# tho-kn/EgoTAP

Measured on AMD Instinct MI355X. Metric: stereo frames/sec (2D->3D lift, B=256, 256x256), higher is better.
Workload: dtype f32; 1 GPU; UnrealEgo 16-joint lifting head (heatmaps [B,90,64,64] -> joints [B,16,3]), forward only, fp32, batch 256 per GPU, inputs resident in HBM; batch_per_gpu=256, global_batch=256, heatmap=64, parallelism=dp1 (batch shards, no collective)

## Files before the change

egotap_amd/csrc/egotap_abi.hip:

```cpp
#include <stdarg.h>
#include <stdio.h>
#include <string.h>

#include <string>
#include <unordered_map>
#include <vector>

#include "attention_f32.h"
#include "common.h"
#include "conv_f32.h"
#include "conv_bf16.h"
#include "gemm_f32.h"
#include "gemm_bf16.h"
#include "gemm_bf16_dma.h"
#include "gemm_f32_dma.h"
#include "attention_bf16.h"
#include "layernorm.h"
#include "metrics.h"
#include "heatmap_synth.h"
#include "pu_chain.h"
#include "gemm_tn_bf16.h"
#include "train_ops.h"
#include "gemm_bf16s.h"
#include "gemm_bf16s64.h"
// ... 773 lines not shown
static hipError_t launch_ln(const float* x, float* y, const float* g, const float* b, int rows, float eps, hipStream_t s) {
    if (rows <= 0) return hipSuccess;
    const int blocks = min((rows + 3) / 4, 256 * 8);
    hipLaunchKernelGGL(layernorm_f32_kernel<1024>, dim3(blocks), dim3(256), 0, s, x, y, g, b, rows, eps);
    return hipGetLastError();
}

#if EGOTAP_IN(0)
static hipError_t gemm_res_ln(Handle* h, const char* role, const float* A, long lda, const float* Wp, const float* bias, float* X, int M, int D, int K,
                              const float* ln_g, const float* ln_b, float* Y, float* P, hipStream_t s) {
    if (D == 1024) {
        const SmallRoute r = gemm_small_route(h, true, M, D, K, D, device_cu_count());
        if ((r.kind == GS_SPLIT_S || r.kind == GS_SPLIT_A) && r.splits > 1) {
            static const std::string kname = "gemm_f32_splitk_kernel<ALoadPlain>+splitk_reduce_res_ln_kernel";
            GemmTimer t(h, s, role, kname.c_str(), 2.0 * M * D * K);
            hipError_t e = r.kind == GS_SPLIT_S ? gemm_f32_splitk_partials<TileS>(ALoadPlain{A, lda}, segmat1(Wp, D, K), P, SPLITK_FLOATS, M, D, K, s, r.splits)
                                                : gemm_f32_splitk_partials<TileA>(ALoadPlain{A, lda}, segmat1(Wp, D, K), P, SPLITK_FLOATS, M, D, K, s, r.splits);
            if (e != hipSuccess) return e;
            hipLaunchKernelGGL(splitk_reduce_res_ln_kernel<1024>, dim3(min((M + 3) / 4, 256 * 8)), dim3(256), 0, s, (const float*)P, bias, (const float*)X, X, ln_g,
                               ln_b, Y, M, r.splits, 1e-12f);
            return hipGetLastError();
        }
    }
    hipError_t e = gemm_small(h, role, ALoadPlain{A, lda}, segmat1(Wp, D, K), EpiBiasRes{segvec1(bias, D), X, D}, X, D, M, D, K, P, s);
    if (e != hipSuccess) return e;
    return launch_ln(X, Y, ln_g, ln_b, M, 1e-12f, s);
}

static ALoadPlain rebase(const ALoadPlain& a, int m0) { return ALoadPlain{a.A + (long)m0 * a.lda, a.lda}; }
static ALoadLive rebase(ALoadLive a, int m0) { a.lr.m0 += m0; return a; }
static EpiBias rebase(const EpiBias& e, int) { return e; }
static EpiBiasGelu rebase(const EpiBiasGelu& e, int) { return e; }
static EpiBiasRes rebase(EpiBiasRes e, int m0) { e.R += (long)m0 * e.ldr; return e; }
static EpiBiasResLive rebase(EpiBiasResLive e, int m0) { e.lr.m0 += m0; return e; }
template <class AL, class Epi>
static hipError_t gemm_rounds(Handle* h, const char* role, const AL& al, const SegMat& W, const Epi& epi, float* C, long ldc, int M, int N, int K,
                              hipStream_t s) {
    const int cus = device_cu_count(), tn = N / 256;
    const long tiles = (long)((M + 255) / 256) * tn;
    const int mh = (int)((tiles / cus) * cus / tn) * 256;
    if (N % 256 == 0 && K % 32 == 0 && mh > 0 && mh < M) {
        const double t_round = K * 0.2319 + 5.0;
        const double t_big = (double)((tiles + cus - 1) / cus) * t_round;
        const double t_split = (double)(((long)(mh / 256) * tn + cus - 1) / cus) * t_round + 4.0 + gemm_f32_direct_estimate_us<TileA>(M - mh, N, K, cus);
        if (t_split < t_big) {
            hipError_t e = gemm_big(h, role, al, W, epi, C, ldc, mh, N, K, s);
            if (e != hipSuccess) return e;
            return gemm<TileA>(h, role, rebase(al, mh), W, rebase(epi, mh), C + (long)mh * ldc, ldc, M - mh, N, K, s);
        }
    }
    return gemm_big(h, role, al, W, epi, C, ldc, M, N, K, s);
}

static bool lift_prune_last(Handle* h, int B) {
#ifdef EGOTAP_ATTN_F32_LIVE
    const int D = h->D, M = B * h->seq, Nq = h->T * h->ppd * h->ppd;
    if (h->precision != EGOTAP_PREC_F32 || h->debug_stop != 0 || h->cfg.vit_layers < 1 || Nq < 32 || Nq >= h->seq || D % 256 != 0) return false;
    const int cus = device_cu_count();
    if (gemm_small_route(h, true, M, 3 * D, D, D, cus, true).kind != GS_BIG || gemm_small_route(h, true, M, D, D, D, cus).kind != GS_BIG ||
        gemm_small_route(h, true, M, 4 * D, D, 4 * D, cus, true).kind != GS_BIG || gemm_small_route(h, true, M, D, 4 * D, D, cus).kind != GS_BIG)
        return false;
    return attention_f32_ksplit(B, h->seq, h->cfg.vit_heads, SPLITK_FLOATS, cus) == 1;
#else
    (void)h; (void)B;
    return false;
#endif
}

static int lift_forward_impl(Handle* h, const float* hm, int B, float* pose, void* ws, size_t ws_bytes, void* stream, bool pose_only,
                             const char* who) {
    EGO_CHECK(h, "null handle");
    if (B == 0) return EGOTAP_OK;
    EGO_CHECK(B > 0 && hm && pose && ws, "%s: null argument or negative batch", who);
    EGO_CHECK(((uintptr_t)hm & 15) == 0 && ((uintptr_t)ws & 255) == 0, "hm must be 16-byte and ws 256-byte aligned");
    int rc = lift_resolve(h);
    if (rc != EGOTAP_OK) return rc;
    const LiftWs w = lift_ws(h, B);
    if (ws_bytes < w.total) {
        egotap_set_error("workspace too small: %zu bytes given, %zu needed for B=%d", ws_bytes, w.total, B);
        return EGOTAP_ERR_WORKSPACE;
    }
    hipStream_t s = (hipStream_t)stream;
    const LiftParams& p = h->lp;
    char* base = (char*)ws;
    auto F = [&](size_t off) { return (float*)(base + off); };
    float *X = F(w.X), *Y = F(w.Y), *QKV = F(w.QKV), *CTX = F(w.CTX), *HID = F(w.HID);
    float* SPK = F(w.SPLITK);
    float *Z1 = F(w.Z1), *Z2 = F(w.Z2), *POSZ = F(w.POSZ), *ROTZ = F(w.ROTZ);
    float *F0 = F(w.F0), *G0 = F(w.G0), *HS0 = F(w.HS0), *F1 = F(w.F1), *G1 = F(w.G1), *HS1 = F(w.HS1);
    float *C0 = F(w.C0), *C1 = F(w.C1), *ZERO = F(w.ZERO), *HPA = F(w.HPA), *HPB = F(w.HPB);
    const int D = h->D, M = B * h->seq, BT = B * h->T, J = h->J, H = h->H, hid = h->hid, JB = J * B;
    const int S = h->cfg.hm_size, HW = S * S;
    using Tile = TileA;

#ifndef EGOTAP_BF16S_MIN_ROWS
#define EGOTAP_BF16S_MIN_ROWS 512
#endif
    constexpr int g_bf16s_min_rows = EGOTAP_BF16S_MIN_ROWS;
    const bool bf16s = h->precision == EGOTAP_PREC_BF16 && D == 1024 && M >= g_bf16s_min_rows && h->wscratch != nullptr && h->seq % 32 == 0 &&
                       h->wscratch_bytes >= (size_t)2 * 2048 * (size_t)(h->ppd * h->ppd * D);
    if (bf16s) {
        __bf16* hmb0 = (__bf16*)HID;
        const long n8 = (long)B * h->C * HW / 8;
        hipLaunchKernelGGL(f32_to_bf16_kernel, dim3((unsigned)((n8 + 255) / 256)), dim3(256), 0, s, hm, hmb0, n8);
        hipLaunchKernelGGL(prep_weight_kernel, dim3((256 + 63) / 64, (D + 63) / 64), dim3(256), 0, s, p.patch_w, h->wscratch, (__bf16*)nullptr, D, 256, (long)D);
        EGO_HIP(zero_fill(SPK, 256, s));
        const XPatch xl{hmb0, (const __bf16*)SPK, h->C, S, h->seq, h->side, h->ppd, h->grid, h->T};
        const SEpiPatchF32 ep{p.patch_b, p.mask_tok, p.pos_emb, X, D, h->seq, h->side, h->ppd, h->grid, h->T};
        EGO_HIP(gemm_bf16s_launch(xl, h->wscratch, 256L, ep, M, D, 256, device_cu_count(), s));
    } else {
        ALoadPatch al{hm, h->C, S, h->seq, h->side, h->ppd, h->grid, h->T};
        if (h->precision == EGOTAP_PREC_F32 && (long)((M + 255) / 256) * (D / 256) >= 160 && (size_t)B * H * 4 >= 1024) {
            EGO_HIP(zero_fill(ZERO, 1024, s));
            al.zeros = ZERO;
        }
        EpiPatch ep{p.patch_b, p.mask_tok, p.pos_emb, D, h->seq, h->side, h->ppd, h->grid, h->T};
        EGO_HIP((gemm_small(h, "patch_embed", al, segmat1(p.patch_w, D, 256), ep, X, D, M, D, 256, SPK, s)));
    }
    if (h->debug_stop == 1) return EGOTAP_OK;
    if (bf16s) {
        __bf16 *Yb = (__bf16*)Y, *QKVb = (__bf16*)QKV, *CTXb = (__bf16*)CTX, *HIDb = (__bf16*)HID, *Wb = h->wscratch;
        float* bias3 = SPK;
        const int cu = device_cu_count();
        auto prep = [&](const float* wsrc, __bf16* dst, int n, int k) {
            hipLaunchKernelGGL(prep_weight_kernel, dim3((k + 63) / 64, (n + 63) / 64), dim3(256), 0, s, wsrc, dst, (__bf16*)nullptr, n, k, (long)n);
        };
        auto ln = [&](const float* gg, const float* bb) {
            hipLaunchKernelGGL(ln_fwd_bf16_kernel<1024>, dim3((M + 3) / 4), dim3(256), 0, s, (const float*)X, Yb, gg, bb, (float*)nullptr, (float*)nullptr, M, 1e-12f);
        };
        for (int i = 0; i < h->cfg.vit_layers; ++i) {
            const auto& L = p.layer[i];
            ln(L.ln1_g, L.ln1_b);
            prep(L.q_w, Wb, D, D); prep(L.k_w, Wb + (size_t)D * D, D, D); prep(L.v_w, Wb + (size_t)2 * D * D, D, D);
            hipLaunchKernelGGL(concat3_kernel, dim3((D + 255) / 256), dim3(256), 0, s, L.q_b, L.k_b, L.v_b, bias3, D);
            EGO_HIP(hipGetLastError());
            EGO_HIP(gemm_bf16s_plain_launch(XPlain{Yb, (long)D}, Wb, (long)D, SEpiBf16{bias3, QKVb, 3L * D}, M, 3 * D, D, cu, s));
            EGO_HIP(attention_bf16s_fwd_launch(QKVb, CTXb, nullptr, B, h->seq, h->cfg.vit_heads, s));
            prep(L.o_w, Wb, D, D);
            EGO_HIP(gemm_bf16s_plain_launch(XPlain{CTXb, (long)D}, Wb, (long)D, SEpiResF32{L.o_b, X, X, (long)D}, M, D, D, cu, s));
            ln(L.ln2_g, L.ln2_b);
            prep(L.up_w, Wb, 4 * D, D);
            EGO_HIP(gemm_bf16s_plain_launch(XPlain{Yb, (long)D}, Wb, (long)D, SEpiGelu{L.up_b, HIDb, 4L * D}, M, 4 * D, D, cu, s));
            prep(L.dn_w, Wb, D, 4 * D);
            EGO_HIP(gemm_bf16s_plain_launch(XPlain{HIDb, 4L * D}, Wb, 4L * D, SEpiResF32{L.dn_b, X, X, (long)D}, M, D, 4 * D, cu, s));
            if (h->debug_stop == 2 + i) return EGOTAP_OK;
        }
        ln(p.lnf_g, p.lnf_b);
        auto bnf = [](const LiftParams::Fc& f, float* out) { return SEpiBnLreluF32{f.b, f.g, f.beta, f.mean, f.var, 1e-5f, 0.2f, out, 2048L}; };
        auto bn = [](const LiftParams::Fc& f) { return EpiBnLrelu{f.b, f.g, f.beta, f.mean, f.var, 1e-5f, 0.2f}; };
        {
            const int K1 = h->ppd * h->ppd * D;
            prep(p.pos_fc[0].w, Wb, 2048, K1);
            const XTokens xt{Yb, h->T, D, h->seq, h->side, h->ppd, h->grid};
            const int sp = gemm_bf16s_ksplit(BT, 2048, K1, cu, SPLITK_FLOATS);
            if (sp > 1) EGO_HIP(gemm_bf16s_splitk_launch(xt, Wb, (long)K1, bnf(p.pos_fc[0], Z1), SPK, sp, BT, 2048, K1, cu, s));
            else EGO_HIP(fc1_nt(h, 0, Yb, Wb, (long)K1, bnf(p.pos_fc[0], Z1), BT, cu, s));
            EGO_HIP((fc_gemm(h, "pos_fc2", ALoadPlain{Z1, 2048}, segmat1(p.pos_fc[1].w, 512, 2048), bn(p.pos_fc[1]), Z2, 512, BT, 512, 2048, SPK, s)));
            EGO_HIP((fc_gemm(h, "pos_fc3", ALoadPlain{Z2, 512}, segmat1(p.pos_fc[2].w, hid, 512), bn(p.pos_fc[2]), POSZ, hid, BT, hid, 512, SPK, s)));
        }
        {
            __bf16* hmb = HIDb;
            const long n8 = (long)B * h->C * HW / 8;
            hipLaunchKernelGGL(f32_to_bf16_kernel, dim3((unsigned)((n8 + 255) / 256)), dim3(256), 0, s, hm, hmb, n8);
            prep(p.rot_fc[0].w, Wb, 2048, 2 * HW);
            EGO_HIP(hipGetLastError());
            const XRot xr{hmb, h->C, J, HW};
            const int sp = gemm_bf16s_ksplit(BT, 2048, 2 * HW, cu, SPLITK_FLOATS);
            if (sp > 1) EGO_HIP(gemm_bf16s_splitk_launch(xr, Wb, 2L * HW, bnf(p.rot_fc[0], Z1), SPK, sp, BT, 2048, 2 * HW, cu, s));
            else EGO_HIP(fc1_nt(h, 1, hmb, Wb, 2L * HW, bnf(p.rot_fc[0], Z1), BT, cu, s));
            EGO_HIP((fc_gemm(h, "rot_fc2", ALoadPlain{Z1, 2048}, segmat1(p.rot_fc[1].w, 512, 2048), bn(p.rot_fc[1]), Z2, 512, BT, 512, 2048, SPK, s)));
            EGO_HIP((fc_gemm(h, "rot_fc3", ALoadPlain{Z2, 512}, segmat1(p.rot_fc[2].w, hid, 512), bn(p.rot_fc[2]), ROTZ, hid, BT, hid, 512, SPK, s)));
        }
    } else {
    const int NL = h->cfg.vit_layers;
    const bool prune = pose_only && lift_prune_last(h, B);
    EGO_HIP(launch_ln(X, Y, NL > 0 ? p.layer[0].ln1_g : p.lnf_g, NL > 0 ? p.layer[0].ln1_b : p.lnf_b, M, 1e-12f, s));
    for (int i = 0; i < NL; ++i) {
        const auto& L = p.layer[i];
#ifdef EGOTAP_ATTN_F32_LIVE
        if (prune && i + 1 == NL) {
            const LiveRows lr{h->seq, h->side, h->ppd, h->grid, h->T};
            const int Nq = h->T * h->ppd * h->ppd, Mc = B * Nq;
            float* Xc = QKV;
            SegMat Wkv; Wkv.p[0] = L.k_w; Wkv.p[1] = L.v_w; Wkv.p[2] = L.v_w; Wkv.seg = D; Wkv.ld = D;
            SegVec bkv; bkv.p[0] = L.k_b; bkv.p[1] = L.v_b; bkv.p[2] = L.v_b; bkv.seg = D;
            EGO_HIP((gemm_big(h, "kv", ALoadPlain{Y, D}, Wkv, EpiBias{bkv}, QKV + D, 3L * D, M, 2 * D, D, s)));
            EGO_HIP((gemm_rounds(h, "q_live", ALoadLive{Y, D, lr}, segmat1(L.q_w, D, D), EpiBias{segvec1(L.q_b, D)}, QKV, 3L * D, Mc, D, D, s)));
            EGO_HIP(attention_f32_live_launch(QKV, 3L * D, Nq, QKV, CTX, B, h->seq, h->cfg.vit_heads, s));
            EGO_HIP((gemm_rounds(h, "attn_out_live", ALoadPlain{CTX, D}, segmat1(L.o_w, D, D), EpiBiasResLive{segvec1(L.o_b, D), X, D, lr}, Xc, D, Mc, D, D, s)));
            EGO_HIP(launch_ln(Xc, Y, L.ln2_g, L.ln2_b, Mc, 1e-12f, s));
            EGO_HIP((gemm_rounds(h, "mlp_up_live", ALoadPlain{Y, D}, segmat1(L.up_w, 4 * D, D), EpiBiasGelu{segvec1(L.up_b, 4 * D)}, HID, 4L * D, Mc, 4 * D, D, s)));
            EGO_HIP((gemm_rounds(h, "mlp_down_live", ALoadPlain{HID, 4L * D}, segmat1(L.dn_w, D, 4 * D), EpiBiasRes{segvec1(L.dn_b, D), Xc, D}, Xc, D, Mc, D, 4 * D, s)));
            EGO_HIP(launch_ln(Xc, Y, p.lnf_g, p.lnf_b, Mc, 1e-12f, s));
            break;
        }
#endif
        {
            SegMat Wqkv; Wqkv.p[0] = L.q_w; Wqkv.p[1] = L.k_w; Wqkv.p[2] = L.v_w; Wqkv.seg = D; Wqkv.ld = D;
            SegVec bqkv; bqkv.p[0] = L.q_b; bqkv.p[1] = L.k_b; bqkv.p[2] = L.v_b; bqkv.seg = D;
            EGO_HIP((gemm_small(h, "qkv", ALoadPlain{Y, D}, Wqkv, EpiBias{bqkv}, QKV, 3L * D, M, 3 * D, D, SPK, s)));
        }
        if (h->precision == EGOTAP_PREC_BF16X3 && h->seq % 32 == 0) EGO_HIP(attention_bf16_launch<3>(QKV, CTX, B, h->seq, h->cfg.vit_heads, s));
        else if (h->precision == EGOTAP_PREC_BF16 && h->seq % 32 == 0) EGO_HIP(attention_bf16_launch<1>(QKV, CTX, B, h->seq, h->cfg.vit_heads, s));
        else EGO_HIP(attention_f32_launch(QKV, CTX, B, h->seq, h->cfg.vit_heads, s, nullptr, SPK, SPLITK_FLOATS, device_cu_count()));
        EGO_HIP(gemm_res_ln(h, "attn_out", CTX, D, L.o_w, L.o_b, X, M, D, D, L.ln2_g, L.ln2_b, Y, SPK, s));
        EGO_HIP((gemm_small(h, "mlp_up", ALoadPlain{Y, D}, segmat1(L.up_w, 4 * D, D), EpiBiasGelu{segvec1(L.up_b, 4 * D)}, HID, 4L * D, M, 4 * D, D, SPK, s)));
        const bool last = i + 1 == NL;
        EGO_HIP(gemm_res_ln(h, "mlp_down", HID, 4L * D, L.dn_w, L.dn_b, X, M, D, 4 * D, last ? p.lnf_g : p.layer[i + 1].ln1_g, last ? p.lnf_b : p.layer[i + 1].ln1_b, Y,
                            SPK, s));
        if (h->debug_stop == 2 + i) return EGOTAP_OK;
    }
    auto bn = [](const LiftParams::Fc& f) { return EpiBnLrelu{f.b, f.g, f.beta, f.mean, f.var, 1e-5f, 0.2f}; };
    const bool skinny_fc1 = BT < SKINNY_ROWS || (h->precision == EGOTAP_PREC_F32 && (long)((BT + 255) / 256) * (2048 / 256) < 100);
    {
        const int K1 = h->ppd * h->ppd * D;
        auto fc1 = [&](const auto& al) -> hipError_t {
            if (skinny_fc1 && BT <= 64)
                return gemm_f32_splitk_launch<TileS>(al, segmat1(p.pos_fc[0].w, 2048, K1), bn(p.pos_fc[0]), Z1, 2048, SPK, SPLITK_FLOATS, BT, 2048, K1, s, device_cu_count());
            if (skinny_fc1)
                return gemm_f32_splitk_launch<TileA>(al, segmat1(p.pos_fc[0].w, 2048, K1), bn(p.pos_fc[0]), Z1, 2048, SPK, SPLITK_FLOATS, BT, 2048, K1, s);
            return gemm_big(h, "pos_fc1", al, segmat1(p.pos_fc[0].w, 2048, K1), bn(p.pos_fc[0]), Z1, 2048, BT, 2048, K1, s);
        };
        if (prune) EGO_HIP(fc1(ALoadPlain{Y, (long)K1}));
        else EGO_HIP(fc1(ALoadTokens{Y, h->T, D, h->seq, h->side, h->ppd, h->grid}));
        EGO_HIP((fc_gemm(h, "pos_fc2", ALoadPlain{Z1, 2048}, segmat1(p.pos_fc[1].w, 512, 2048), bn(p.pos_fc[1]), Z2, 512, BT, 512, 2048, SPK, s)));
        EGO_HIP((fc_gemm(h, "pos_fc3", ALoadPlain{Z2, 512}, segmat1(p.pos_fc[2].w, hid, 512), bn(p.pos_fc[2]), POSZ, hid, BT, hid, 512, SPK, s)));
    }
    {
        ALoadRot al{hm, h->C, J, HW};
        if (skinny_fc1 && BT <= 64)
            EGO_HIP((gemm_f32_splitk_launch<TileS>(al, segmat1(p.rot_fc[0].w, 2048, 2L * HW), bn(p.rot_fc[0]), Z1, 2048, SPK, SPLITK_FLOATS, BT, 2048, 2 * HW, s, device_cu_count())));
        else if (skinny_fc1)
            EGO_HIP((gemm_f32_splitk_launch<TileA>(al, segmat1(p.rot_fc[0].w, 2048, 2L * HW), bn(p.rot_fc[0]), Z1, 2048, SPK, SPLITK_FLOATS, BT, 2048, 2 * HW, s)));
        else
            EGO_HIP((gemm_big(h, "rot_fc1", al, segmat1(p.rot_fc[0].w, 2048, 2L * HW), bn(p.rot_fc[0]), Z1, 2048, BT, 2048, 2 * HW, s)));
        EGO_HIP((fc_gemm(h, "rot_fc2", ALoadPlain{Z1, 2048}, segmat1(p.rot_fc[1].w, 512, 2048), bn(p.rot_fc[1]), Z2, 512, BT, 512, 2048, SPK, s)));
        EGO_HIP((fc_gemm(h, "rot_fc3", ALoadPlain{Z2, 512}, segmat1(p.rot_fc[2].w, hid, 512), bn(p.rot_fc[2]), ROTZ, hid, BT, hid, 512, SPK, s)));
    }
    }
    const int x = 2 * hid, NF0 = H + x;
    ALoadStereo xs{POSZ, B, J, hid};
    EGO_HIP((fc_gemm(h, "pu0_x2f", xs, segmat1(p.x2f0_w, NF0, x), EpiBias{segvec1(p.x2f0_b, NF0)}, F0, NF0, JB, NF0, x, SPK, s)));
    EGO_HIP((fc_gemm(h, "pu0_x2h", xs, segmat1(p.x2h0_w, 4 * H, x), EpiBias{segvec1(p.x2h0_b, 4 * H)}, G0, 4L * H, JB, 4 * H, x, SPK, s)));
    {
        ALoadStereoGated bs{ALoadStereo{ROTZ, B, J, hid}, F0, NF0, H};
        EGO_HIP((fc_gemm(h, "pu0_b2h", bs, segmat1(p.b2h0_w, 4 * H, x), EpiBiasRes{segvec1(p.b2h0_b, 4 * H), G0, 4L * H}, G0, 4L * H, JB, 4 * H, x, SPK, s)));
    }
    EGO_HIP(zero_fill(C0, (size_t)(w.ZERO - w.C0) + al256((size_t)B * H * 4), s));
    pu_chain_probe(h);
    unsigned* FAULT = (unsigned*)(base + w.FAULT);
    const PuChain ch0{F0, (long)B * NF0, NF0, G0, (long)B * 4 * H, nullptr, p.h2h0_w, p.h2h0_b, nullptr, 0, HS0, (long)B * H, HPA, (long)B * H, B, H, J,
                      FAULT, h->pu_fault_dev};
    if (!pu_chain_launch(s, h->pu_resident[0], h->pu_resident[1], ch0, B, h->pu_debug_drop))
// ... 2467 lines not shown
```

egotap_amd/csrc/gemm_f32.h:

```cpp
#pragma once
#include "common.h"
#include <type_traits>

struct ALoadPlain {
    const float* A;
    long lda;
    struct Row { const float* p; };
    __device__ __forceinline__ Row row(int m) const { return Row{A + (long)m * lda}; }
    __device__ __forceinline__ f32x4 load(const Row& r, int k) const { return *(const f32x4*)(r.p + k); }
    static constexpr bool HAS_PTR = true;
    __device__ __forceinline__ const float* ptr(const Row& r, int k) const { return r.p + k; }
    __host__ bool dma_ok() const { return lda % 4 == 0 && lda < (1L << 21) && ((uintptr_t)A & 15) == 0; }
};

struct ALoadPatch {
    const float* hm;
    int C, S, seq, side, ppd, grid, T;
    const float* zeros = nullptr;
    struct Row { const float* p; };
    static constexpr bool HAS_PTR = true;
    __device__ __forceinline__ const float* ptr(const Row& r, int k) const { return r.p ? r.p + (k >> 4) * S + (k & 15) : zeros + k; }
    __host__ bool dma_ok() const { return zeros != nullptr && S % 4 == 0 && ((uintptr_t)hm & 15) == 0 && ((uintptr_t)zeros & 15) == 0; }
    __device__ __forceinline__ Row row(int m) const {
        const int b = m / seq, tok = m - b * seq;
// ... 3 lines not shown
        return Row{hm + ((long)(b * C + cell) * S + (pr % ppd) * 16) * S + (pc % ppd) * 16};
    }
    __device__ __forceinline__ f32x4 load(const Row& r, int k) const {
        if (r.p == nullptr) return f32x4{0.f, 0.f, 0.f, 0.f};
        return *(const f32x4*)(r.p + (k >> 4) * S + (k & 15));
    }
};

struct ALoadTokens {
    const float* Y;
    int T, D, seq, side, ppd, grid;
    struct Row { const float* p; };
    __device__ __forceinline__ Row row(int m) const {
        const int b = m / T, i = m - b * T;
        return Row{Y + ((long)b * seq + (long)(ppd * (i / grid)) * side + ppd * (i % grid)) * D};
    }
    __device__ __forceinline__ f32x4 load(const Row& r, int k) const {
        const int s = k / D, c = k - s * D;
        const int prl = s / ppd, pcl = s - prl * ppd;
        return *(const f32x4*)(r.p + (long)(prl * side + pcl) * D + c);
    }
    static constexpr bool HAS_PTR = true;
    __device__ __forceinline__ const float* ptr(const Row& r, int k) const {
        const int s = k / D, c = k - s * D;
        const int prl = s / ppd, pcl = s - prl * ppd;
        return r.p + (long)(prl * side + pcl) * D + c;
    }
    __host__ bool dma_ok() const { return D % 4 == 0 && ((uintptr_t)Y & 15) == 0; }
};

struct LiveRows {
    int seq, side, ppd, grid, T;
    int m0 = 0;
    __host__ __device__ __forceinline__ long phys(int m) const {
        m += m0;
        const int pp = ppd * ppd, L = T * pp;
        const int b = m / L, r = m - b * L, i = r / pp, s = r - i * pp;
        const int pr = (i / grid) * ppd + s / ppd, pc = (i % grid) * ppd + s % ppd;
        return (long)b * seq + pr * side + pc;
    }
};
struct ALoadLive {
    const float* A;
    long lda;
    LiveRows lr;
    struct Row { const float* p; };
    __device__ __forceinline__ Row row(int m) const { return Row{A + lr.phys(m) * lda}; }
    __device__ __forceinline__ f32x4 load(const Row& r, int k) const { return *(const f32x4*)(r.p + k); }
    static constexpr bool HAS_PTR = true;
    __device__ __forceinline__ const float* ptr(const Row& r, int k) const { return r.p + k; }
    __host__ bool dma_ok() const { return lda % 4 == 0 && lda < (1L << 21) && ((uintptr_t)A & 15) == 0; }
};

struct ALoadRot {
    const float* hm;
    int C, J, HW;
    struct Row { const float* p; };
    __device__ __forceinline__ Row row(int m) const {
        const int T = 2 * J;
        const int b = m / T, t = m - b * T;
        const int eye = t / J, j = t - eye * J;
        return Row{hm + (long)(b * C + 2 * J + eye * 2 * J + j) * HW};
    }
    __device__ __forceinline__ f32x4 load(const Row& r, int k) const {
        const int cs = k / HW;
        return *(const f32x4*)(r.p + (long)cs * J * HW + (k - cs * HW));
    }
    static constexpr bool HAS_PTR = true;
    __device__ __forceinline__ const float* ptr(const Row& r, int k) const {
        const int cs = k / HW;
        return r.p + (long)cs * J * HW + (k - cs * HW);
    }
    __host__ bool dma_ok() const { return HW % 4 == 0 && ((uintptr_t)hm & 15) == 0; }
};

struct ALoadStereo {
    static constexpr bool HAS_PTR = false;
    const float* Z;
    int B, J, hid;
    struct Row { const float* p; };
    __device__ __forceinline__ Row row(int m) const {
        const int t = m / B, b = m - t * B;
        return Row{Z + ((long)b * 2 * J + t) * hid};
    }
    __device__ __forceinline__ f32x4 load(const Row& r, int k) const {
        const int eye = k / hid;
        return *(const f32x4*)(r.p + (long)eye * J * hid + (k - eye * hid));
    }
};

struct ALoadStereoGated {
    static constexpr bool HAS_PTR = false;
    ALoadStereo z;
    const float* F;
    int ldf, fcol0;
    struct Row { ALoadStereo::Row r; const float* f; };
    __device__ __forceinline__ Row row(int m) const { return Row{z.row(m), F + (long)m * ldf + fcol0}; }
    __device__ __forceinline__ f32x4 load(const Row& r, int k) const {
        f32x4 v = z.load(r.r, k);
        const f32x4 g = *(const f32x4*)(r.f + k);
#pragma unroll
        for (int i = 0; i < 4; ++i) v[i] *= 1.0f / (1.0f + expf(-g[i]));
        return v;
    }
};

// ... 55 lines not shown
        f32x4 o;
#pragma unroll
        for (int i = 0; i < 4; ++i) {
            const float x = acc[i] + c.b[i];
            o[i] = gelu_erf(x);
        }
        return o;
    }
};
struct EpiBnLrelu {
    const float *bias, *gamma, *beta, *mean, *var;
    float eps, slope;
    struct Col { float b, mu, sc, sh; };
    __device__ __forceinline__ Col col(int n) const {
        return Col{bias[n], mean[n], gamma[n] / sqrtf(var[n] + eps), beta[n]};
    }
    __device__ __forceinline__ float apply(float acc, const Col& c, int m, int n) const {
        const float y = (acc + c.b - c.mu) * c.sc + c.sh;
        return y > 0.f ? y : slope * y;
    }
    struct Col4 { Col c[4]; };
    __device__ __forceinline__ Col4 col4(int n0) const { return Col4{{col(n0), col(n0 + 1), col(n0 + 2), col(n0 + 3)}}; }
    static constexpr bool HAS_RES = false;
    __device__ __forceinline__ f32x4 res4(int m, int n0) const { return f32x4{0.f, 0.f, 0.f, 0.f}; }
    __device__ __forceinline__ f32x4 apply4(f32x4 acc, const Col4& c, f32x4 res, int m, int n0) const {
        f32x4 o;
#pragma unroll
        for (int i = 0; i < 4; ++i) o[i] = apply(acc[i], c.c[i], m, n0 + i);
        return o;
    }
};
struct EpiPatch {
    const float *bias, *mask_tok, *pos;
    int D, seq, side, ppd, grid, T;
    struct Col { float b, mt; };
    __device__ __forceinline__ Col col(int n) const { return Col{bias[n], mask_tok[n]}; }
    __device__ __forceinline__ float apply(float acc, const Col& c, int m, int n) const {
        const int tok = m % seq;
        const int pr = tok / side, pc = tok - pr * side;
        const bool dummy = (pr / ppd) * grid + pc / ppd >= T;
        return (dummy ? c.mt : acc + c.b) + pos[(long)tok * D + n];
    }
    struct Col4 { f32x4 b, mt; };
    __device__ __forceinline__ Col4 col4(int n0) const { return Col4{*(const f32x4*)(bias + n0), *(const f32x4*)(mask_tok + n0)}; }
    static constexpr bool HAS_RES = true;
    __device__ __forceinline__ f32x4 res4(int m, int n0) const { return *(const f32x4*)(pos + (long)(m % seq) * D + n0); }
    __device__ __forceinline__ f32x4 apply4(f32x4 acc, const Col4& c, f32x4 res, int m, int n0) const {
        const int tok = m % seq;
        const int pr = tok / side, pc = tok - pr * side;
        const bool dummy = (pr / ppd) * grid + pc / ppd >= T;
        return (dummy ? c.mt : acc + c.b) + res;
    }
};

struct EpiNone {
    struct Col {};
    __device__ __forceinline__ Col col(int n) const { return Col{}; }
    __device__ __forceinline__ float apply(float acc, const Col& c, int m, int n) const { return acc; }
    struct Col4 {};
    __device__ __forceinline__ Col4 col4(int n0) const { return Col4{}; }
    static constexpr bool HAS_RES = false;
    __device__ __forceinline__ f32x4 res4(int m, int n0) const { return f32x4{0.f, 0.f, 0.f, 0.f}; }
    __device__ __forceinline__ f32x4 apply4(f32x4 acc, const Col4& c, f32x4 res, int m, int n0) const { return acc; }
};
struct EpiAccum {
    const float* R;
    long ldr;
    struct Col {};
    __device__ __forceinline__ Col col(int n) const { return Col{}; }
    __device__ __forceinline__ float apply(float acc, const Col& c, int m, int n) const { return acc + R[(long)m * ldr + n]; }
    struct Col4 {};
    __device__ __forceinline__ Col4 col4(int n0) const { return Col4{}; }
    static constexpr bool HAS_RES = true;
    __device__ __forceinline__ f32x4 res4(int m, int n0) const { return *(const f32x4*)(R + (long)m * ldr + n0); }
    __device__ __forceinline__ f32x4 apply4(f32x4 acc, const Col4& c, f32x4 res, int m, int n0) const { return acc + res; }
};
struct EpiBiasGeluSave {
    SegVec bias;
    float* Z;
    long ldz;
    struct Col { float b; };
    __device__ __forceinline__ Col col(int n) const { return Col{bias.at(n)}; }
    __device__ __forceinline__ float apply(float acc, const Col& c, int m, int n) const {
        const float x = acc + c.b;
        Z[(long)m * ldz + n] = x;
        return gelu_erf(x);
    }
    struct Col4 { f32x4 b; };
    __device__ __forceinline__ Col4 col4(int n0) const { return Col4{bias.at4(n0)}; }
    static constexpr bool HAS_RES = false;
    __device__ __forceinline__ f32x4 res4(int m, int n0) const { return f32x4{0.f, 0.f, 0.f, 0.f}; }
    __device__ __forceinline__ f32x4 apply4(f32x4 acc, const Col4& c, f32x4 res, int m, int n0) const {
        const f32x4 x = acc + c.b;
        *(f32x4*)(Z + (long)m * ldz + n0) = x;
        f32x4 o;
#pragma unroll
        for (int i = 0; i < 4; ++i) o[i] = gelu_erf(x[i]);
        return o;
    }
};
struct EpiGeluGrad {
    const float* Z;
    long ldz;
    __device__ __forceinline__ static float dgelu(float z) {
        return dgelu_erf(z);
    }
// ... 664 lines not shown
```

egotap_amd/csrc/gemm_f32_dma.h:

```cpp
#pragma once
#include <type_traits>
#include "gemm_f32.h"
#include "lds_dma.h"

struct DmaF32Cfg {
    static constexpr int BM = 256, BN = 256, BK = 16, WM = 4, WN = 2, THREADS = 512, NS = 4, TM = 2, TN = 4;
    static constexpr int ROWB = 64;
    static constexpr int STAGE = (BM + BN) * ROWB;
    static constexpr int ELD = 36, EPATCH = 16 * ELD * 4;
    static constexpr int LDS_BYTES = NS * STAGE + (THREADS / 64) * EPATCH;
    static_assert(LDS_BYTES <= 160 * 1024, "LDS budget");
};

template <class ALoad, class Epi>
__global__ __launch_bounds__(DmaF32Cfg::THREADS, 2) void gemm_f32_dma_kernel(ALoad al, SegMat W, Epi epi, float* C,
                                                                          long ldc, int M, int N, int K, int tiles_m, int tiles_n) {
    using Cfg = DmaF32Cfg;
    constexpr int BM = Cfg::BM, BN = Cfg::BN, BK = Cfg::BK, NS = Cfg::NS, TM = Cfg::TM, TN = Cfg::TN, ROWB = Cfg::ROWB, ELD = Cfg::ELD;
    extern __shared__ __attribute__((aligned(16))) char smem_dmaf[];
    const int tid = threadIdx.x, lane = tid & 63, wid = tid >> 6;
    const int wm = wid / Cfg::WN, wn = wid % Cfg::WN;
    const int l31 = lane & 31, lh = lane >> 5;
    float* Es = (float*)(smem_dmaf + NS * Cfg::STAGE + wid * Cfg::EPATCH);

    const int ntiles = tiles_m * tiles_n, nb = gridDim.x, x8 = blockIdx.x & 7, jb = blockIdx.x >> 3;
    const int nbx = (nb >> 3) + (x8 < (nb & 7) ? 1 : 0);
    const int q8 = ntiles >> 3, r8 = ntiles & 7;
    const int lo_t = x8 < r8 ? x8 * (q8 + 1) : r8 * (q8 + 1) + (x8 - r8) * q8;
    const int cnt = q8 + (x8 < r8 ? 1 : 0);
    const int my_n = cnt > jb ? (cnt - jb + nbx - 1) / nbx : 0;
    const int KT = K / BK;
    const int total = my_n * KT;
    if (total == 0) return;
    auto tile_of = [&](int i, int& tm, int& tn) __attribute__((always_inline)) {
        const int lin = lo_t + jb + i * nbx;
        const int per_group = 8 * tiles_n;
        const int g = lin / per_group, first = g * 8;
        const int gsz = min(tiles_m - first, 8);
        const int in = lin - g * per_group;
        tm = first + in % gsz;
        tn = in / gsz;
    };

    const int drow = lane >> 2, dchunk = (lane & 3) ^ (lane >> 4);
    typename ALoad::Row ra0, ra1;
    const float *pb0, *pb1;
#ifdef EGOTAP_F32_DMA_FLAT
    constexpr bool SBA = false, SBW = false;
#else
    constexpr bool SBA = std::is_same<ALoad, ALoadPlain>::value, SBW = true;
#endif
    unsigned long long abase = 0, wbase = 0;
    unsigned ao0 = 0, ao1 = 0;
    auto uniform64 = [](const void* p) __attribute__((always_inline)) { return lds_dma_base(p); };
    const unsigned wo0 = (unsigned)(((long)(wid * 16 + drow) * W.ld + dchunk * 4) * 4), wo1 = (unsigned)(((long)((wid + 8) * 16 + drow) * W.ld + dchunk * 4) * 4);
    int l_tile = 0, l_kt = 0;
    auto set_rows = [&](int i) __attribute__((always_inline)) {
        int tm, tn;
        tile_of(i, tm, tn);
        if constexpr (SBA) {
            abase = uniform64(al.A + (long)tm * BM * al.lda);
            const long ld = al.lda * 4;
            ao0 = (unsigned)((long)(min(tm * BM + wid * 16 + drow, M - 1) - tm * BM) * ld + dchunk * 16);
            ao1 = (unsigned)((long)(min(tm * BM + (wid + 8) * 16 + drow, M - 1) - tm * BM) * ld + dchunk * 16);
        } else {
        ra0 = al.row(min(tm * BM + wid * 16 + drow, M - 1));
        ra1 = al.row(min(tm * BM + (wid + 8) * 16 + drow, M - 1));
        }
        const int n0 = tn * BN, sidx = n0 / W.seg;
        const float* wp = (sidx == 0 ? W.p[0] : (sidx == 1 ? W.p[1] : W.p[2])) + (long)(n0 - sidx * W.seg) * W.ld;
        if constexpr (SBW) wbase = uniform64(wp);
        else {
        pb0 = wp + (long)(wid * 16 + drow) * W.ld + dchunk * 4;
        pb1 = wp + (long)((wid + 8) * 16 + drow) * W.ld + dchunk * 4;
        }
    };
    set_rows(0);
    const unsigned lds0 = (unsigned)(size_t)(__attribute__((address_space(3))) char*)smem_dmaf;
    auto dma1 = [&](const float* g, unsigned lds_addr) __attribute__((always_inline)) {
        asm volatile("s_mov_b32 m0, %1\n\ts_nop 0\n\tglobal_load_lds_dwordx4 %0, off" ::"v"(g), "s"(__builtin_amdgcn_readfirstlane(lds_addr)) : "memory");
    };
    auto dma1s = [&](unsigned voff, unsigned long long sbase, unsigned lds_addr) __attribute__((always_inline)) {
        asm volatile("s_mov_b32 m0, %2\n\ts_nop 0\n\tglobal_load_lds_dwordx4 %0, %1" ::"v"(voff), "s"(sbase), "s"(__builtin_amdgcn_readfirstlane(lds_addr)) : "memory");
    };
    auto dma_part = [&](int st, int part) __attribute__((always_inline)) {
        const unsigned sa = lds0 + st * Cfg::STAGE + wid * 1024;
        const int k0 = l_kt * BK;
        if (part == 0) { if constexpr (SBA) dma1s(ao0, abase + (unsigned long long)k0 * 4, sa); else dma1(al.ptr(ra0, k0 + dchunk * 4), sa); }
        else if (part == 1) { if constexpr (SBA) dma1s(ao1, abase + (unsigned long long)k0 * 4, sa + 8 * 1024); else dma1(al.ptr(ra1, k0 + dchunk * 4), sa + 8 * 1024); }
        else if (part == 2) { if constexpr (SBW) dma1s(wo0, wbase + (unsigned long long)k0 * 4, sa + BM * ROWB); else dma1(pb0 + k0, sa + BM * ROWB); }
        else { if constexpr (SBW) dma1s(wo1, wbase + (unsigned long long)k0 * 4, sa + BM * ROWB + 8 * 1024); else dma1(pb1 + k0, sa + BM * ROWB + 8 * 1024); }
    };
    auto dma_advance = [&]() __attribute__((always_inline)) {
        if (l_tile < my_n && ++l_kt == KT) {
            l_kt = 0;
            if (++l_tile < my_n) set_rows(l_tile);
            else l_kt = KT - 1;
        }
    };
    auto dma = [&](int st) __attribute__((always_inline)) {
        dma_part(st, 0); dma_part(st, 1); dma_part(st, 2); dma_part(st, 3);
        dma_advance();
    };

    f32x16 acc[TM][TN];
#pragma unroll
    for (int i = 0; i < TM; ++i)
#pragma unroll
        for (int j = 0; j < TN; ++j)
#pragma unroll
            for (int r = 0; r < 16; ++r) acc[i][j][r] = 0.f;
    const int sw = (l31 >> 2) & 3;
    const int f0 = l31 * ROWB + ((lh ^ sw) << 4), f1 = l31 * ROWB + (((2 + lh) ^ sw) << 4);
    const int a_base = (wm * (TM * 32)) * ROWB, b_base = (BM + wn * (TN * 32)) * ROWB;

    int c_tile = 0, c_kt = 0;
    auto epilogue = [&](auto full_tag) __attribute__((always_inline)) {
        constexpr bool FULL = decltype(full_tag)::value;
        int tm, tn;
        tile_of(c_tile, tm, tn);
        const int er = lane >> 3, ec = (lane & 7) * 4;
        const int nb0 = tn * BN + wn * (TN * 32) + ec, mb0 = tm * BM + wm * (TM * 32) + er;
        f32x4 rs[2] = {{0.f, 0.f, 0.f, 0.f}, {0.f, 0.f, 0.f, 0.f}}, rn[2] = {{0.f, 0.f, 0.f, 0.f}, {0.f, 0.f, 0.f, 0.f}};
        if (Epi::HAS_RES) {
#pragma unroll
            for (int s2 = 0; s2 < 2; ++s2) rs[s2] = epi.res4(min(mb0 + s2 * 8, M - 1), nb0);
        }
        typename Epi::Col4 cc = epi.col4(nb0), cn = cc;
#pragma unroll
        for (int q = 0; q < TN * TM * 2; ++q) {
            const int j = q / (TM * 2), i = (q / 2) % TM, hf = q & 1;
            const int n0 = nb0 + j * 32, mb = mb0 + i * 32;
            if (q + 1 < TN * TM * 2 && (q + 1) / (TM * 2) != j) cn = epi.col4(nb0 + ((q + 1) / (TM * 2)) * 32);
            if (Epi::HAS_RES && q + 1 < TN * TM * 2) {
                const int jn = (q + 1) / (TM * 2), in = ((q + 1) / 2) % TM, hn = (q + 1) & 1;
#pragma unroll
                for (int s2 = 0; s2 < 2; ++s2) rn[s2] = epi.res4(min(mb0 + in * 32 + hn * 16 + s2 * 8, M - 1), nb0 + jn * 32);
            }
#pragma unroll
            for (int r = 8 * hf; r < 8 * hf + 8; ++r) Es[((r & 3) + 8 * ((r >> 2) & 1) + 4 * lh) * ELD + l31] = acc[i][j][r];
#pragma unroll
            for (int r = 8 * hf; r < 8 * hf + 8; ++r) acc[i][j][r] = 0.f;
#pragma unroll
            for (int s2 = 0; s2 < 2; ++s2) {
                const int m = mb + hf * 16 + s2 * 8;
                if (FULL || m < M) {
                    const f32x4 o = epi.apply4(*(const f32x4*)(Es + (s2 * 8 + er) * ELD + ec), cc, rs[s2], m, n0);
                    *(f32x4*)(C + (long)m * ldc + n0) = o;
                }
            }
            if (Epi::HAS_RES) { rs[0] = rn[0]; rs[1] = rn[1]; }
            cc = cn;
        }
    };

    dma(0);
    dma(1);
    dma(2);
    asm volatile("s_waitcnt vmcnt(8)" ::: "memory");
    __syncthreads();
    f32x4 a0[TM], b0[TN], a1[TM], b1[TN];
#pragma unroll
    for (int i = 0; i < TM; ++i) a0[i] = *(const f32x4*)(smem_dmaf + a_base + i * 32 * ROWB + f0);
#pragma unroll
    for (int j = 0; j < TN; ++j) b0[j] = *(const f32x4*)(smem_dmaf + b_base + j * 32 * ROWB + f0);
    int st = 0;
    bool after_epi = false;
    for (int gs = 0; gs < total; ++gs) {
        const char* sa = smem_dmaf + st * Cfg::STAGE;
        const int st1 = st + 1 == NS ? 0 : st + 1;
#pragma unroll
        for (int q = 0; q < 6; ++q) {
            acc[q & 1][q >> 1] = __builtin_amdgcn_mfma_f32_32x32x2f32(a0[q & 1][0], b0[q >> 1][0], acc[q & 1][q >> 1], 0, 0, 0);
            __builtin_amdgcn_sched_barrier(0);
            if (q < TM) a1[q] = *(const f32x4*)(sa + a_base + q * 32 * ROWB + f1);
            else b1[q - TM] = *(const f32x4*)(sa + b_base + (q - TM) * 32 * ROWB + f1);
            __builtin_amdgcn_sched_barrier(0);
        }
#pragma unroll
        for (int u = 0; u < 4; ++u)
#pragma unroll
            for (int j = 0; j < TN; ++j)
#pragma unroll
                for (int i = 0; i < TM; ++i)
                    if (u > 0 || j >= 3) acc[i][j] = __builtin_amdgcn_mfma_f32_32x32x2f32(a0[i][u], b0[j][u], acc[i][j], 0, 0, 0);
        if (!after_epi) asm volatile("s_waitcnt vmcnt(4)" ::: "memory");
        after_epi = false;
        __syncthreads();
        const int sd = st == 0 ? NS - 1 : st - 1;
        const char* sn = smem_dmaf + st1 * Cfg::STAGE;
        __builtin_amdgcn_sched_barrier(0);
#pragma unroll
        for (int q = 0; q < 4; ++q) {
            acc[q & 1][q >> 1] = __builtin_amdgcn_mfma_f32_32x32x2f32(a1[q & 1][0], b1[q >> 1][0], acc[q & 1][q >> 1], 0, 0, 0);
            __builtin_amdgcn_sched_barrier(0);
            dma_part(sd, q);
            __builtin_amdgcn_sched_barrier(0);
        }
        dma_advance();
#pragma unroll
        for (int q = 0; q < 6; ++q) {
// ... 53 lines not shown
```

egotap_amd/csrc/layernorm.h:

```cpp
#pragma once
#include "common.h"

__device__ __forceinline__ float wave_sum(float v) {
#pragma unroll
    for (int o = 32; o > 0; o >>= 1) v += __shfl_xor(v, o, 64);
    return v;
}
__device__ __forceinline__ float wave_max(float v) {
#pragma unroll
    for (int o = 32; o > 0; o >>= 1) v = fmaxf(v, __shfl_xor(v, o, 64));
    return v;
}

template <int D>
__global__ __launch_bounds__(256) void layernorm_f32_kernel(const float* __restrict__ X, float* __restrict__ Y,
                                                            const float* __restrict__ gamma,
                                                            const float* __restrict__ beta, int rows, float eps) {
    static_assert(D % 256 == 0, "D must be a multiple of 256");
    constexpr int V = D / 256;
    const int lane = threadIdx.x & 63;
    const int wave = (blockIdx.x * blockDim.x + threadIdx.x) >> 6;
    const int nwaves = (gridDim.x * blockDim.x) >> 6;
    f32x4 g[V], b[V];
#pragma unroll
    for (int i = 0; i < V; ++i) {
        g[i] = *(const f32x4*)(gamma + (i * 64 + lane) * 4);
        b[i] = *(const f32x4*)(beta + (i * 64 + lane) * 4);
    }
    for (int r = wave; r < rows; r += nwaves) {
        const float* x = X + (long)r * D;
        f32x4 v[V];
#pragma unroll
        for (int i = 0; i < V; ++i) v[i] = *(const f32x4*)(x + (i * 64 + lane) * 4);
        float s = 0.f;
#pragma unroll
        for (int i = 0; i < V; ++i) s += (v[i][0] + v[i][1]) + (v[i][2] + v[i][3]);
        const float mu = wave_sum(s) * (1.0f / D);
        float q = 0.f;
#pragma unroll
        for (int i = 0; i < V; ++i)
#pragma unroll
            for (int c = 0; c < 4; ++c) {
                const float d = v[i][c] - mu;
                q += d * d;
            }
        const float rstd = 1.0f / sqrtf(wave_sum(q) * (1.0f / D) + eps);
        float* y = Y + (long)r * D;
#pragma unroll
        for (int i = 0; i < V; ++i) {
            f32x4 o;
#pragma unroll
            for (int c = 0; c < 4; ++c) o[c] = (v[i][c] - mu) * rstd * g[i][c] + b[i][c];
            *(f32x4*)(y + (i * 64 + lane) * 4) = o;
        }
    }
}

template <int D>
__global__ __launch_bounds__(256) void splitk_reduce_res_ln_kernel(const float* __restrict__ P, const float* __restrict__ bias, const float* R, float* X,
                                                                   const float* __restrict__ gamma, const float* __restrict__ beta, float* __restrict__ Y,
                                                                   int rows, int splits, float eps) {
    static_assert(D % 256 == 0, "D must be a multiple of 256");
    constexpr int V = D / 256;
    const int lane = threadIdx.x & 63;
    const int wave = (blockIdx.x * blockDim.x + threadIdx.x) >> 6;
    const int nwaves = (gridDim.x * blockDim.x) >> 6;
    for (int r = wave; r < rows; r += nwaves) {
        f32x4 v[V];
#pragma unroll
        for (int i = 0; i < V; ++i) {
            const int n = (i * 64 + lane) * 4;
            f32x4 acc{0.f, 0.f, 0.f, 0.f};
            for (int k = 0; k < splits; ++k) acc += *(const f32x4*)(P + ((long)k * rows + r) * D + n);
            v[i] = acc + *(const f32x4*)(bias + n) + *(const f32x4*)(R + (long)r * D + n);
            *(f32x4*)(X + (long)r * D + n) = v[i];
        }
        float s = 0.f;
#pragma unroll
        for (int i = 0; i < V; ++i) s += (v[i][0] + v[i][1]) + (v[i][2] + v[i][3]);
        const float mu = wave_sum(s) * (1.0f / D);
        float q = 0.f;
#pragma unroll
        for (int i = 0; i < V; ++i)
#pragma unroll
            for (int c = 0; c < 4; ++c) {
                const float d = v[i][c] - mu;
                q += d * d;
            }
        const float rstd = 1.0f / sqrtf(wave_sum(q) * (1.0f / D) + eps);
#pragma unroll
        for (int i = 0; i < V; ++i) {
            const int n = (i * 64 + lane) * 4;
            const f32x4 g = *(const f32x4*)(gamma + n), b = *(const f32x4*)(beta + n);
            f32x4 o;
#pragma unroll
            for (int c = 0; c < 4; ++c) o[c] = (v[i][c] - mu) * rstd * g[c] + b[c];
            *(f32x4*)(Y + (long)r * D + n) = o;
        }
    }
}
```

Measured before the change: 2876 stereo frames/s.

## Compute layer-0 LayerNorm and QKV once for batch-invariant dummy tokens

Masked dummy tokens come out of the patch embedding identical in every batch item, because they depend only on the mask token and positional embedding. For the first ViT layer, LayerNorm and the QKV GEMM now run only on batch 0's full sequence plus the live tokens of the other items. A row-remapping loader and a scattering epilogue in the f32 DMA GEMM support this, and a small kernel then copies the dummy QKV rows to the remaining batch items. The aim is to cut redundant layer-0 FLOPs and memory traffic. In exchange the change adds an extra broadcast launch and per-row index arithmetic inside the GEMM address setup.

After: 2900 stereo frames/s, median of 6. No clear change (+0.8%).

```diff
diff --git a/egotap_amd/csrc/egotap_abi.hip b/egotap_amd/csrc/egotap_abi.hip
--- a/egotap_amd/csrc/egotap_abi.hip
+++ b/egotap_amd/csrc/egotap_abi.hip
@@ -849,6 +849,36 @@
     return gemm_big(h, role, al, W, epi, C, ldc, M, N, K, s);
 }
 
+template <class AL, class Epi>
+static hipError_t gemm_rep(Handle* h, const char* role, const ALoadRep<AL>& al, const SegMat& W, const EpiRep<Epi>& epi, float* C, long ldc,
+                           int M, int N, int K, hipStream_t s) {
+    static const std::string kdma = std::string("gemm_f32_dma_kernel<256x256x16,ALoadRep<") + AlName<AL>::v + ">,EpiRep<" + EpiName<Epi>::v + ">>";
+    GemmTimer t(h, s, role, kdma.c_str(), 2.0 * M * N * K);
+    return gemm_f32_dma_launch(al, W, epi, C, ldc, M, N, K, device_cu_count(), s);
+}
+static __global__ __launch_bounds__(256) void bcast_dummy_rows_kernel(float* A, long ld, int w4, RepRows rr, long total) {
+    const long i = (long)blockIdx.x * blockDim.x + threadIdx.x;
+    if (i >= total) return;
+    const int nd = rr.dummies();
+    const long r = i / w4;
+    const int c = (int)(i - r * w4), d = (int)(r % nd);
+    const long b = 1 + r / nd, tok = rr.dummy_tok(d);
+    ((f32x4*)(A + (b * rr.seq + tok) * ld))[c] = ((const f32x4*)(A + tok * ld))[c];
+}
+static hipError_t bcast_dummy_rows(float* A, long ld, int width, const RepRows& rr, int B, hipStream_t s) {
+    const long total = (long)(B - 1) * rr.dummies() * (width / 4);
+    if (total <= 0) return hipSuccess;
+    if (width % 4 != 0 || ld % 4 != 0 || ((uintptr_t)A & 15)) return hipErrorInvalidValue;
+    hipLaunchKernelGGL(bcast_dummy_rows_kernel, dim3((unsigned)((total + 255) / 256)), dim3(256), 0, s, A, ld, width / 4, rr, total);
+    return hipGetLastError();
+}
+static hipError_t launch_ln_rows(const float* x, float* y, const float* g, const float* b, const RepRows& rr, int rows, float eps, hipStream_t s) {
+    if (rows <= 0) return hipSuccess;
+    const int blocks = min((rows + 3) / 4, 256 * 8);
+    hipLaunchKernelGGL((layernorm_f32_rows_kernel<1024, RepRows>), dim3(blocks), dim3(256), 0, s, x, y, g, b, rows, eps, rr);
+    return hipGetLastError();
+}
+
 static bool lift_prune_last(Handle* h, int B) {
 #ifdef EGOTAP_ATTN_F32_LIVE
     const int D = h->D, M = B * h->seq, Nq = h->T * h->ppd * h->ppd;
@@ -896,6 +926,10 @@
     constexpr int g_bf16s_min_rows = EGOTAP_BF16S_MIN_ROWS;
     const bool bf16s = h->precision == EGOTAP_PREC_BF16 && D == 1024 && M >= g_bf16s_min_rows && h->wscratch != nullptr && h->seq % 32 == 0 &&
                        h->wscratch_bytes >= (size_t)2 * 2048 * (size_t)(h->ppd * h->ppd * D);
+    const int NL = h->cfg.vit_layers;
+    const bool prune = pose_only && lift_prune_last(h, B);
+    const RepRows rr{h->seq, h->side, h->ppd, h->grid, h->T};
+    const bool rep0 = prune && NL >= 2 && rr.dummies() > 0;
     if (bf16s) {
         __bf16* hmb0 = (__bf16*)HID;
         const long n8 = (long)B * h->C * HW / 8;
@@ -969,9 +1003,8 @@
             EGO_HIP((fc_gemm(h, "rot_fc3", ALoadPlain{Z2, 512}, segmat1(p.rot_fc[2].w, hid, 512), bn(p.rot_fc[2]), ROTZ, hid, BT, hid, 512, SPK, s)));
         }
     } else {
-    const int NL = h->cfg.vit_layers;
-    const bool prune = pose_only && lift_prune_last(h, B);
-    EGO_HIP(launch_ln(X, Y, NL > 0 ? p.layer[0].ln1_g : p.lnf_g, NL > 0 ? p.layer[0].ln1_b : p.lnf_b, M, 1e-12f, s));
+    if (rep0) EGO_HIP(launch_ln_rows(X, Y, p.layer[0].ln1_g, p.layer[0].ln1_b, rr, (int)rr.rows(B), 1e-12f, s));
+    else EGO_HIP(launch_ln(X, Y, NL > 0 ? p.layer[0].ln1_g : p.lnf_g, NL > 0 ? p.layer[0].ln1_b : p.lnf_b, M, 1e-12f, s));
     for (int i = 0; i < NL; ++i) {
         const auto& L = p.layer[i];
 #ifdef EGOTAP_ATTN_F32_LIVE
@@ -995,7 +1028,12 @@
         {
             SegMat Wqkv; Wqkv.p[0] = L.q_w; Wqkv.p[1] = L.k_w; Wqkv.p[2] = L.v_w; Wqkv.seg = D; Wqkv.ld = D;
             SegVec bqkv; bqkv.p[0] = L.q_b; bqkv.p[1] = L.k_b; bqkv.p[2] = L.v_b; bqkv.seg = D;
-            EGO_HIP((gemm_small(h, "qkv", ALoadPlain{Y, D}, Wqkv, EpiBias{bqkv}, QKV, 3L * D, M, 3 * D, D, SPK, s)));
+            if (rep0 && i == 0) {
+                EGO_HIP((gemm_rep(h, "qkv", ALoadRep<ALoadPlain>{ALoadPlain{Y, D}, rr}, Wqkv, EpiRep<EpiBias>{EpiBias{bqkv}, rr}, QKV, 3L * D, (int)rr.rows(B), 3 * D, D, s)));
+                EGO_HIP(bcast_dummy_rows(QKV, 3L * D, 3 * D, rr, B, s));
+            } else {
+                EGO_HIP((gemm_small(h, "qkv", ALoadPlain{Y, D}, Wqkv, EpiBias{bqkv}, QKV, 3L * D, M, 3 * D, D, SPK, s)));
+            }
         }
         if (h->precision == EGOTAP_PREC_BF16X3 && h->seq % 32 == 0) EGO_HIP(attention_bf16_launch<3>(QKV, CTX, B, h->seq, h->cfg.vit_heads, s));
         else if (h->precision == EGOTAP_PREC_BF16 && h->seq % 32 == 0) EGO_HIP(attention_bf16_launch<1>(QKV, CTX, B, h->seq, h->cfg.vit_heads, s));
diff --git a/egotap_amd/csrc/gemm_f32.h b/egotap_amd/csrc/gemm_f32.h
--- a/egotap_amd/csrc/gemm_f32.h
+++ b/egotap_amd/csrc/gemm_f32.h
@@ -79,6 +79,43 @@
     __host__ bool dma_ok() const { return lda % 4 == 0 && lda < (1L << 21) && ((uintptr_t)A & 15) == 0; }
 };
 
+struct RepRows {
+    int seq, side, ppd, grid, T;
+    __host__ __device__ __forceinline__ int live() const { return T * ppd * ppd; }
+    __host__ __device__ __forceinline__ int dummies() const { return seq - live(); }
+    __host__ __device__ __forceinline__ long rows(int B) const { return seq + (long)(B - 1) * live(); }
+    __host__ __device__ __forceinline__ int live_tok(int l) const {
+        const int full = (T / grid) * ppd * side, w = (T % grid) * ppd;
+        if (l < full) return l;
+        const int l2 = l - full;
+        return ((T / grid) * ppd + l2 / w) * side + l2 % w;
+    }
+    __host__ __device__ __forceinline__ int dummy_tok(int d) const {
+        const int fr = T / grid, w = (T % grid) * ppd, part = w > 0 ? ppd * (side - w) : 0;
+        if (d < part) return (fr * ppd + d / (side - w)) * side + w + d % (side - w);
+        return (fr * ppd + (w > 0 ? ppd : 0)) * side + (d - part);
+    }
+    __host__ __device__ __forceinline__ long phys(int m) const {
+        if (m < seq) return m;
+        const int r = m - seq, L = live(), b = r / L;
+        return (long)(b + 1) * seq + live_tok(r - b * L);
+    }
+};
+template <class AL>
+struct ALoadRep {
+    AL in;
+    RepRows rr;
+    using Row = typename AL::Row;
+    static constexpr bool HAS_PTR = true;
+    static_assert(AL::HAS_PTR, "ALoadRep: the inner loader must be address math");
+    __device__ __forceinline__ Row row(int m) const { return in.row((int)rr.phys(m)); }
+    __device__ __forceinline__ f32x4 load(const Row& r, int k) const { return in.load(r, k); }
+    __device__ __forceinline__ const float* ptr(const Row& r, int k) const { return in.ptr(r, k); }
+    __host__ bool dma_ok() const { return in.dma_ok(); }
+};
+template <class AL> struct is_rep_plain : std::false_type {};
+template <> struct is_rep_plain<ALoadRep<ALoadPlain>> : std::true_type {};
+
 struct ALoadRot {
     const float* hm;
     int C, J, HW;
@@ -240,6 +277,23 @@
         return (dummy ? c.mt : acc + c.b) + res;
     }
 };
+template <class E>
+struct EpiRep {
+    E in;
+    RepRows rr;
+    using Col = typename E::Col;
+    using Col4 = typename E::Col4;
+    static constexpr bool HAS_RES = E::HAS_RES;
+    __device__ __forceinline__ long out_row(int m) const { return rr.phys(m); }
+    __device__ __forceinline__ Col col(int n) const { return in.col(n); }
+    __device__ __forceinline__ Col4 col4(int n0) const { return in.col4(n0); }
+    __device__ __forceinline__ f32x4 res4(int m, int n0) const { return in.res4((int)rr.phys(m), n0); }
+    __device__ __forceinline__ f32x4 apply4(f32x4 acc, const Col4& c, f32x4 res, int m, int n0) const {
+        return in.apply4(acc, c, res, (int)rr.phys(m), n0);
+    }
+};
+template <class E> struct epi_scatters : std::false_type {};
+template <class E> struct epi_scatters<EpiRep<E>> : std::true_type {};
 
 struct EpiNone {
     struct Col {};
diff --git a/egotap_amd/csrc/gemm_f32_dma.h b/egotap_amd/csrc/gemm_f32_dma.h
--- a/egotap_amd/csrc/gemm_f32_dma.h
+++ b/egotap_amd/csrc/gemm_f32_dma.h
@@ -48,8 +48,9 @@
 #ifdef EGOTAP_F32_DMA_FLAT
     constexpr bool SBA = false, SBW = false;
 #else
-    constexpr bool SBA = std::is_same<ALoad, ALoadPlain>::value, SBW = true;
+    constexpr bool SBA = std::is_same<ALoad, ALoadPlain>::value || is_rep_plain<ALoad>::value, SBW = true;
 #endif
+    constexpr bool REP = SBA && is_rep_plain<ALoad>::value;
     unsigned long long abase = 0, wbase = 0;
     unsigned ao0 = 0, ao1 = 0;
     auto uniform64 = [](const void* p) __attribute__((always_inline)) { return lds_dma_base(p); };
@@ -58,7 +59,12 @@
     auto set_rows = [&](int i) __attribute__((always_inline)) {
         int tm, tn;
         tile_of(i, tm, tn);
-        if constexpr (SBA) {
+        if constexpr (REP) {
+            const long p0 = al.rr.phys(tm * BM), ld = al.in.lda * 4;
+            abase = uniform64(al.in.A + p0 * al.in.lda);
+            ao0 = (unsigned)((al.rr.phys(min(tm * BM + wid * 16 + drow, M - 1)) - p0) * ld + dchunk * 16);
+            ao1 = (unsigned)((al.rr.phys(min(tm * BM + (wid + 8) * 16 + drow, M - 1)) - p0) * ld + dchunk * 16);
+        } else if constexpr (SBA) {
             abase = uniform64(al.A + (long)tm * BM * al.lda);
             const long ld = al.lda * 4;
             ao0 = (unsigned)((long)(min(tm * BM + wid * 16 + drow, M - 1) - tm * BM) * ld + dchunk * 16);
@@ -86,8 +92,12 @@
     auto dma_part = [&](int st, int part) __attribute__((always_inline)) {
         const unsigned sa = lds0 + st * Cfg::STAGE + wid * 1024;
         const int k0 = l_kt * BK;
-        if (part == 0) { if constexpr (SBA) dma1s(ao0, abase + (unsigned long long)k0 * 4, sa); else dma1(al.ptr(ra0, k0 + dchunk * 4), sa); }
-        else if (part == 1) { if constexpr (SBA) dma1s(ao1, abase + (unsigned long long)k0 * 4, sa + 8 * 1024); else dma1(al.ptr(ra1, k0 + dchunk * 4), sa + 8 * 1024); }
+        auto asb = [&]() __attribute__((always_inline)) {
+            if constexpr (REP) return lds_dma_base(abase + (unsigned long long)k0 * 4);
+            else return abase + (unsigned long long)k0 * 4;
+        };
+        if (part == 0) { if constexpr (SBA) dma1s(ao0, asb(), sa); else dma1(al.ptr(ra0, k0 + dchunk * 4), sa); }
+        else if (part == 1) { if constexpr (SBA) dma1s(ao1, asb(), sa + 8 * 1024); else dma1(al.ptr(ra1, k0 + dchunk * 4), sa + 8 * 1024); }
         else if (part == 2) { if constexpr (SBW) dma1s(wo0, wbase + (unsigned long long)k0 * 4, sa + BM * ROWB); else dma1(pb0 + k0, sa + BM * ROWB); }
         else { if constexpr (SBW) dma1s(wo1, wbase + (unsigned long long)k0 * 4, sa + BM * ROWB + 8 * 1024); else dma1(pb1 + k0, sa + BM * ROWB + 8 * 1024); }
     };
@@ -146,7 +156,9 @@
                 const int m = mb + hf * 16 + s2 * 8;
                 if (FULL || m < M) {
                     const f32x4 o = epi.apply4(*(const f32x4*)(Es + (s2 * 8 + er) * ELD + ec), cc, rs[s2], m, n0);
-                    *(f32x4*)(C + (long)m * ldc + n0) = o;
+                    long mo = m;
+                    if constexpr (epi_scatters<Epi>::value) mo = epi.out_row(m);
+                    *(f32x4*)(C + mo * ldc + n0) = o;
                 }
             }
             if (Epi::HAS_RES) { rs[0] = rn[0]; rs[1] = rn[1]; }
diff --git a/egotap_amd/csrc/layernorm.h b/egotap_amd/csrc/layernorm.h
--- a/egotap_amd/csrc/layernorm.h
+++ b/egotap_amd/csrc/layernorm.h
@@ -10,6 +10,34 @@
 #pragma unroll
     for (int o = 32; o > 0; o >>= 1) v = fmaxf(v, __shfl_xor(v, o, 64));
     return v;
+}
+
+template <int D>
+__device__ __forceinline__ void ln_row(const float* __restrict__ x, float* __restrict__ y, const f32x4* g, const f32x4* b, float eps, int lane) {
+    constexpr int V = D / 256;
+    f32x4 v[V];
+#pragma unroll
+    for (int i = 0; i < V; ++i) v[i] = *(const f32x4*)(x + (i * 64 + lane) * 4);
+    float s = 0.f;
+#pragma unroll
+    for (int i = 0; i < V; ++i) s += (v[i][0] + v[i][1]) + (v[i][2] + v[i][3]);
+    const float mu = wave_sum(s) * (1.0f / D);
+    float q = 0.f;
+#pragma unroll
+    for (int i = 0; i < V; ++i)
+#pragma unroll
+        for (int c = 0; c < 4; ++c) {
+            const float d = v[i][c] - mu;
+            q += d * d;
+        }
+    const float rstd = 1.0f / sqrtf(wave_sum(q) * (1.0f / D) + eps);
+#pragma unroll
+    for (int i = 0; i < V; ++i) {
+        f32x4 o;
+#pragma unroll
+        for (int c = 0; c < 4; ++c) o[c] = (v[i][c] - mu) * rstd * g[i][c] + b[i][c];
+        *(f32x4*)(y + (i * 64 + lane) * 4) = o;
+    }
 }
 
 template <int D>
@@ -27,32 +55,26 @@
         g[i] = *(const f32x4*)(gamma + (i * 64 + lane) * 4);
         b[i] = *(const f32x4*)(beta + (i * 64 + lane) * 4);
     }
+    for (int r = wave; r < rows; r += nwaves) ln_row<D>(X + (long)r * D, Y + (long)r * D, g, b, eps, lane);
+}
+
+template <int D, class Rows>
+__global__ __launch_bounds__(256) void layernorm_f32_rows_kernel(const float* __restrict__ X, float* __restrict__ Y,
+                                                                 const float* __restrict__ gamma, const float* __restrict__ beta,
+                                                                 int rows, float eps, Rows map) {
+    constexpr int V = D / 256;
+    const int lane = threadIdx.x & 63;
+    const int wave = (blockIdx.x * blockDim.x + threadIdx.x) >> 6;
+    const int nwaves = (gridDim.x * blockDim.x) >> 6;
+    f32x4 g[V], b[V];
+#pragma unroll
+    for (int i = 0; i < V; ++i) {
+        g[i] = *(const f32x4*)(gamma + (i * 64 + lane) * 4);
+        b[i] = *(const f32x4*)(beta + (i * 64 + lane) * 4);
+    }
     for (int r = wave; r < rows; r += nwaves) {
-        const float* x = X + (long)r * D;
-        f32x4 v[V];
-#pragma unroll
-        for (int i = 0; i < V; ++i) v[i] = *(const f32x4*)(x + (i * 64 + lane) * 4);
-        float s = 0.f;
-#pragma unroll
-        for (int i = 0; i < V; ++i) s += (v[i][0] + v[i][1]) + (v[i][2] + v[i][3]);
-        const float mu = wave_sum(s) * (1.0f / D);
-        float q = 0.f;
-#pragma unroll
-        for (int i = 0; i < V; ++i)
-#pragma unroll
-            for (int c = 0; c < 4; ++c) {
-                const float d = v[i][c] - mu;
-                q += d * d;
-            }
-        const float rstd = 1.0f / sqrtf(wave_sum(q) * (1.0f / D) + eps);
-        float* y = Y + (long)r * D;
-#pragma unroll
-        for (int i = 0; i < V; ++i) {
-            f32x4 o;
-#pragma unroll
-            for (int c = 0; c < 4; ++c) o[c] = (v[i][c] - mu) * rstd * g[i][c] + b[i][c];
-            *(f32x4*)(y + (i * 64 + lane) * 4) = o;
-        }
+        const long pr = map.phys(r);
+        ln_row<D>(X + pr * D, Y + pr * D, g, b, eps, lane);
     }
 }
 
```
